# chaiyujin/sdfa-2019

Measured on AMD Instinct MI355X. Metric: animation frames/s/node (10 s@16 kHz clips); max|Δdgrad| vs CPU ref, higher is better.
Workload: dtype f32

## Files before the change

sdfa-2019_amd/csrc/api_core.cpp:

```cpp
#include "../../include/sdfa_stream.h"
#include "host.h"

#include <climits>
#include <cstdio>
#include <cstring>
#include <string>

static thread_local std::string g_err;

int sdfa_failv(int code, const char *fmt, va_list ap) {
    char buf[512];
    vsnprintf(buf, sizeof buf, fmt, ap);
    g_err = buf;
    return code;
}

int sdfa_fail(int code, const char *fmt, ...) {
    va_list ap;
    va_start(ap, fmt);
    sdfa_failv(code, fmt, ap);
    va_end(ap);
    return code;
}

thread_local int g_sdfa_mel_fft_radix4 = 0;
thread_local int g_sdfa_gather_plain_order = 0;
thread_local int g_sdfa_frontend_two_kernel = 0;
thread_local int g_sdfa_frontend_stream_block = 0;
thread_local int g_sdfa_frontend_stream_slots = 0;
thread_local int g_sdfa_frontend_stream_spin_max = 0;
thread_local int g_sdfa_frontend_stream_phases = 0;
thread_local int g_sdfa_frontend_t_major = 0;
extern thread_local int g_sdfa_gemm_variant;
thread_local int g_sdfa_freq_lstm_shape = 0;
thread_local int g_sdfa_pca_lds = 0;
thread_local int g_sdfa_pca_fp32 = 0;
thread_local int g_sdfa_conv_fp32 = 0;
thread_local int g_sdfa_time_lstm_split = 0;
thread_local int g_sdfa_time_lstm_handoff = 0;
thread_local int g_sdfa_time_lstm_timeout_us = 0;
thread_local int g_sdfa_share_gx0_off = 0;
thread_local int g_sdfa_encoder_dedup_off = 0;
thread_local int g_sdfa_attn_unfused = 0;

extern "C" {

int sdfa_abi_version(void) { return SDFA_ABI_VERSION; }
int sdfa_stream_abi_version(void) { return SDFA_STREAM_ABI_VERSION; }
const char *sdfa_last_error(void) { return g_err.c_str(); }

int sdfa_debug_set_option(const char *name, int value) {
    struct Option { const char *name; int *var; int lo = INT_MIN, hi = INT_MAX; const char *accepts = nullptr; };
    thread_local const Option options[] = {
        {"attn_unfused", &g_sdfa_attn_unfused},
        {"share_gx0_off", &g_sdfa_share_gx0_off},
        {"encoder_dedup_off", &g_sdfa_encoder_dedup_off},
        {"frontend_two_kernel", &g_sdfa_frontend_two_kernel},
        {"frontend_stream_phases", &g_sdfa_frontend_stream_phases},
        {"frontend_stream_spin_max", &g_sdfa_frontend_stream_spin_max, 0, INT_MAX, "0 (default) or a positive poll count"},
        {"frontend_stream_block", &g_sdfa_frontend_stream_block, 0, 256, "0 (default) or 1..256 frames"},
        {"frontend_stream_slots", &g_sdfa_frontend_stream_slots, 0, 256, "0 (default) or 1..256 workgroups per block"},
        {"gather_plain_order", &g_sdfa_gather_plain_order},
        {"mel_fft_radix4", &g_sdfa_mel_fft_radix4},
        {"frontend_t_major", &g_sdfa_frontend_t_major},
        {"time_lstm_timeout_us", &g_sdfa_time_lstm_timeout_us},
        {"time_lstm_handoff", &g_sdfa_time_lstm_handoff},
        {"time_lstm_split", &g_sdfa_time_lstm_split},
        {"gemm_variant", &g_sdfa_gemm_variant},
        {"freq_lstm_shape", &g_sdfa_freq_lstm_shape},
        {"pca_lds", &g_sdfa_pca_lds},
        {"conv_fp32", &g_sdfa_conv_fp32},
        {"pca_fp32", &g_sdfa_pca_fp32},
    };
    for (const Option &o : options)
        if (name && !strcmp(name, o.name)) {
            if (value < o.lo || value > o.hi) return sdfa_fail(SDFA_EINVAL, "%s: %s", o.name, o.accepts);
            *o.var = value;
            return SDFA_OK;
        }
    return sdfa_fail(SDFA_EINVAL, "unknown option '%s'", name ? name : "(null)");
}

}
```

sdfa-2019_amd/csrc/api_forward.cpp:

```cpp
#include "host.h"
#include "kernels.h"
#include "model.h"

#include <algorithm>

extern thread_local int g_sdfa_freq_lstm_shape, g_sdfa_pca_lds, g_sdfa_pca_fp32, g_sdfa_conv_fp32, g_sdfa_share_gx0_off, g_sdfa_attn_unfused, g_sdfa_encoder_dedup_off;

namespace {

constexpr int64_t CT_WORDS = 2048, CT_FLAGS = 16, ST_WORDS = SDFA_WS_STATUS_BYTES / 4;

struct Ws {
    int64_t P1, X3, HF, Z, GX, H0, H1, KP, QC, QP, ZK, SH, ZU, total;
    int64_t TRUNK, A0, A1, COEF;
    int64_t CT_FREQ, CT_PCA, CT_FLAG;
};

Ws layout(int64_t Nc, bool keep) {
    const int64_t Mc = 64 * Nc;
    Ws w{};
    int64_t o = 0;
    auto take = [&](int64_t n) { int64_t r = o; o += round_up(n, 64); return r; };
    take(ST_WORDS);
    if (keep) {
        w.P1 = take(2048 * Mc); w.X3 = take(2048 * Mc); w.HF = take((int64_t)HF_SLAB_ROWS * 4 * Mc); w.Z = take(256 * Mc);
        w.GX = take(2048 * Mc); w.H0 = take(512 * Mc); w.H1 = take(512 * Mc); w.KP = take(128 * Mc);
    } else {
        const int64_t A = take(2048 * Mc);
        const int64_t B = take(2048 * Mc);
        w.HF = take((int64_t)HF_SLAB_ROWS * 4 * Mc);
        w.P1 = A; w.GX = A;
        w.X3 = B; w.Z = B; w.H0 = B + 256 * Mc; w.H1 = B + 768 * Mc; w.KP = B + 1280 * Mc;
    }
    w.QC = take(512 * Nc); w.QP = take(128 * Nc); w.ZK = take(512 * Nc);
    const int64_t R = take(2560 * Nc);
    w.TRUNK = R; w.A0 = R + 512 * Nc; w.A1 = R + 1024 * Nc; w.COEF = R + 1280 * Nc;
    w.SH = take(sdfa_share_table_words(Nc) + 111);
    w.ZU = keep ? take(256 * Mc) : w.P1;
    const int64_t CT = take(CT_WORDS);
    w.CT_FREQ = CT; w.CT_PCA = CT + 1; w.CT_FLAG = CT + CT_FLAGS;
    w.total = o;
    return w;
}

int64_t capacity(int64_t bytes, bool keep) {
    const int64_t per128 = layout(128, keep).total * 4;
    int64_t nc = (bytes / per128 + 2) * 128;
    while (nc > 0 && layout(nc, keep).total * 4 > bytes) nc -= 128;
    return nc;
}

struct Prof {
    const sdfa_model *m;
    hipStream_t s;
    hipEvent_t pending = nullptr;
    void begin(const char *stage) {
        if (!m->profile) return;
        sdfa_model::Ev e; e.stage = stage;
        (void)hipEventCreate(&e.a); (void)hipEventCreate(&e.b);
        (void)hipEventRecord(e.a, s);
        pending = e.b;
        std::lock_guard<std::mutex> lk(m->ev_mu);
        m->events.push_back(e);
    }
    void end() {
        if (!m->profile || !pending) return;
        (void)hipEventRecord(pending, s);
        pending = nullptr;
    }
};

GemmArgs gemm_fc(const sdfa_model::Fc &fc, const float *Q, int64_t ldq, float *D, int64_t Nc, const int64_t *spk, int64_t nreal) {
    GemmArgs g = sdfa_gemm_k4(fc.w, fc.Ppad, Q, ldq, D, Nc, fc.K);
    g.bias = fc.b; g.cond_w = fc.cw; g.cond_idx = fc.cw ? spk : nullptr;
    g.Pstore = fc.Pstore; g.Qreal = nreal; g.act = fc.act;
    return g;
}

}

extern "C" {

int64_t sdfa_workspace_bytes(const sdfa_model *m, int64_t max_frames) {
    if (!m || max_frames <= 0) return sdfa_fail(SDFA_EINVAL, "workspace_bytes: bad argument");
    return layout(round_up(max_frames, 128), m->keep).total * 4;
}

int sdfa_debug_keep_intermediates(sdfa_model *m, int on) {
    if (!m) return sdfa_fail(SDFA_EINVAL, "null model");
    m->keep = on != 0;
    return SDFA_OK;
}

int sdfa_profile_enable(sdfa_model *m, int on) {
    if (!m) return sdfa_fail(SDFA_EINVAL, "null model");
    std::lock_guard<std::mutex> lk(m->ev_mu);
    m->profile = on != 0;
    for (auto &e : m->events) { (void)hipEventDestroy(e.a); (void)hipEventDestroy(e.b); }
    m->events.clear();
    return SDFA_OK;
}

float sdfa_profile_ms(const sdfa_model *m, const char *stage) {
    if (!m || !stage) return (float)sdfa_fail(SDFA_EINVAL, "profile_ms: bad argument");
    float total = 0.f;
    bool any = false;
    std::lock_guard<std::mutex> lk(m->ev_mu);
    for (auto &e : m->events)
        if (e.stage == stage) {
            float ms = 0.f;
            if (hipEventSynchronize(e.b) != hipSuccess || hipEventElapsedTime(&ms, e.a, e.b) != hipSuccess)
                return (float)sdfa_fail(SDFA_EHIP, "profile_ms: event query failed");
            total += ms; any = true;
        }
    return any ? total : (float)sdfa_fail(SDFA_EINVAL, "profile_ms: no such stage '%s'", stage);
}

int sdfa_profile_reset(sdfa_model *m) { return m ? sdfa_profile_enable(m, m->profile) : sdfa_fail(SDFA_EINVAL, "null model"); }

enum { STAGE_BODY = 0, STAGE_ATTENTION = 1, STAGE_REGRESSOR = 2 };
static int stage_terms(const sdfa_model *m, int stage) {
    switch (m->precision) {
    case SDFA_PREC_BF16_ATTENTION: return stage == STAGE_ATTENTION ? 1 : 0;
    case SDFA_PREC_BF16X3_ATTENTION: return stage == STAGE_ATTENTION ? 3 : 0;
    case SDFA_PREC_BF16X6: return 6;
    case SDFA_PREC_BF16X3: return 3;
    case SDFA_PREC_BF16: return 1;
    default: return 0;
    }
}

int sdfa_model_set_precision(sdfa_model *m, int mode) {
    if (!m) return sdfa_fail(SDFA_EINVAL, "null model");
    if (mode < SDFA_PREC_FP32 || mode > SDFA_PREC_BF16X6) return sdfa_fail(SDFA_EINVAL, "unknown precision mode %d", mode);
    m->precision = mode;
    return SDFA_OK;
}

int sdfa_model_precision(const sdfa_model *m) { return m ? m->precision : SDFA_EINVAL; }

int sdfa_model_set_reserved_cus(sdfa_model *m, int k) {
    if (!m) return sdfa_fail(SDFA_EINVAL, "null model");
    if (k < 0 || k > 128) return sdfa_fail(SDFA_EINVAL, "reserved_cus must be in [0, 128], got %d", k);
    m->reserved_cus.store(k);
    return SDFA_OK;
}

static int encoder_impl(const sdfa_model *m, const float *d_audio_feat, int64_t n_frames, const int32_t *d_frame_clip,
                        const int64_t *d_frame_start, int hop, float *d_z, float *d_align, void *d_workspace,
                        int64_t workspace_bytes, void *stream) {
    if (!m || !m->finalized) return sdfa_fail(SDFA_ESTATE, "encoder_forward: model not finalised");
    if (n_frames == 0) return SDFA_OK;
    if (!d_audio_feat || !d_z || !d_workspace || n_frames < 0) return sdfa_fail(SDFA_EINVAL, "encoder_forward: bad argument");
    if (((uintptr_t)d_workspace | (uintptr_t)d_audio_feat | (uintptr_t)d_z) & 15) return sdfa_fail(SDFA_EINVAL, "encoder_forward: pointers must be 16-byte aligned");
    if ((uintptr_t)d_align & 3) return sdfa_fail(SDFA_EINVAL, "encoder_forward: d_align must be 4-byte aligned");
    const int64_t cap = capacity(workspace_bytes, m->keep);
    if (cap < 128) return sdfa_fail(SDFA_ENOSPACE, "encoder_forward: workspace of %lld bytes holds no 128-frame chunk", (long long)workspace_bytes);
    hipStream_t s = (hipStream_t)stream;
    Prof pf{m, s};
    float *ws = (float *)d_workspace;
    for (int64_t f0 = 0; f0 < n_frames; f0 += cap) {
        const int64_t N = std::min(cap, n_frames - f0);
        const int64_t Nc = round_up(N, 128), Mc = 64 * Nc;
        const Ws w = layout(Nc, m->keep);
        ConvArgs ca{};
        ca.audio_feat = d_audio_feat + f0 * (64 * 128 * 3); ca.N = N; ca.Nc = Nc; ca.Mc = Mc;
        ca.w1 = m->w1; ca.b1 = m->b1; ca.s1 = m->s1; ca.t1 = m->t1; ca.P1 = ws + w.P1;
        ca.w2 = m->w2; ca.b2 = m->b2; ca.s2 = m->s2; ca.t2 = m->t2;
        ca.w3 = m->w3; ca.b3 = m->b3; ca.s3 = m->s3; ca.t3 = m->t3; ca.X3 = ws + w.X3;
        const bool table = d_frame_clip != nullptr;
        const bool share = table || (!m->keep && !g_sdfa_encoder_dedup_off);
        const int64_t *d_ulimit = nullptr;
        int32_t *col_to_u = nullptr;
        if (share) {
            ShareArgs sa{};
            sa.N = N; sa.Nc = Nc; sa.Mc = Mc;
            sdfa_share_carve(sa, reinterpret_cast<int32_t *>(ws + w.SH));
            pf.begin("share_map");
            if (table) {
                sa.frame_clip = d_frame_clip + f0; sa.frame_start = d_frame_start + f0; sa.hop = hop;
                sa.t_lo = 6; sa.t_hi = 58;
                HIP_TRY(sdfa_launch_share_map(sa, s));
            } else {
                sa.feat = ca.audio_feat;
                sa.hash = reinterpret_cast<uint64_t *>(ws + w.HF); sa.linked = sa.hash + Mc;
                HIP_TRY(sdfa_launch_share_map_content(sa, s));
            }
            pf.end();
            d_ulimit = sa.counts + 1; col_to_u = sa.col_to_u;
            ca.col_src = sa.col_src; ca.col_limit = d_ulimit;
        }
        const int conv_terms = g_sdfa_conv_fp32 ? 0 : stage_terms(m, STAGE_BODY);
        if (m->keep && conv_terms) {
            pf.begin("conv1"); HIP_TRY(sdfa_launch_conv1(ca, s)); pf.end();
            ca.wb = m->cv_wb; ca.terms = conv_terms;
            pf.begin("conv23"); HIP_TRY(sdfa_launch_conv123(ca, s)); pf.end();
        } else if (m->keep) {
            pf.begin("conv1"); HIP_TRY(sdfa_launch_conv1(ca, s)); pf.end();
            pf.begin("conv23"); HIP_TRY(sdfa_launch_conv23(ca, s)); pf.end();
        } else {
            ca.wb = m->cv_wb; ca.terms = conv_terms;
            pf.begin("conv23"); HIP_TRY(sdfa_launch_conv123(ca, s)); pf.end();
        }

        const int fl_terms = stage_terms(m, STAGE_BODY);
        FreqLstmArgs fa{ws + w.X3, m->fl_w, m->fl_b, ws + w.HF, Mc, d_ulimit, m->fl_wb, fl_terms, reinterpret_cast<int *>(ws + w.CT_FREQ),
                        g_sdfa_freq_lstm_shape ? g_sdfa_freq_lstm_shape : (fl_terms ? 0 : m->freq_shape.load()), m->reserved_cus.load()};
        pf.begin("freq_lstm"); HIP_TRY(sdfa_launch_freq_lstm(fa, s)); pf.end();

        GemmArgs g = sdfa_gemm_k4(m->fp_w, 256, ws + w.HF, Mc, ws + w.Z, Mc, 8192);
        g.bias = m->fp_b; g.q_tile_major = 1; g.q_slab_rows = HF_SLAB_ROWS;
        g.terms = stage_terms(m, STAGE_BODY);
        g.reserve_cus = m->reserved_cus.load();
        if (share) { g.D = ws + w.ZU; g.q_limit = d_ulimit; }
        pf.begin("freq_proj"); HIP_TRY(sdfa_launch_gemm(g, s)); pf.end();
        const bool share_gx0 = share && !m->keep && stage_terms(m, STAGE_BODY) == 0 && !g_sdfa_share_gx0_off;
        if (share && !share_gx0) {
            pf.begin("share_expand"); HIP_TRY(sdfa_launch_expand_cols(ws + w.ZU, col_to_u, ws + w.Z, 64, Mc, s)); pf.end();
        }

        const float *xin = share_gx0 ? ws + w.ZU : ws + w.Z;
        float *hout[2] = {ws + w.H0, ws + w.H1};
        const char *gxn[2] = {"gx0", "gx1"}, *lsn[2] = {"lstm0", "lstm1"};
        for (int l = 0; l < 2; ++l) {
            const bool mapped = share_gx0 && l == 0;
            float *gx = mapped ? ws + w.HF : ws + w.GX;
            GemmArgs gi = sdfa_gemm_k4(m->gx_w[l], 2048, xin, Mc, gx, Mc, l == 0 ? 256 : 512);
            gi.terms = stage_terms(m, STAGE_BODY);
            gi.reserve_cus = m->reserved_cus.load();
            if (mapped) gi.q_limit = d_ulimit;
            pf.begin(gxn[l]); HIP_TRY(sdfa_launch_gemm(gi, s)); pf.end();
            TimeLstmArgs ta{gx, m->tl_w[l], hout[l], Nc, Mc, m->tl_wb[l], stage_terms(m, STAGE_BODY),
                            reinterpret_cast<unsigned *>(ws + w.CT_FLAG), CT_WORDS - CT_FLAGS, m->tl_w16[l],
                            reinterpret_cast<unsigned *>(ws), m->reserved_cus.load(), mapped ? col_to_u : nullptr};
            pf.begin(lsn[l]); HIP_TRY(sdfa_launch_time_lstm(ta, s)); pf.end();
            xin = hout[l];
        }
        const int at_terms = stage_terms(m, STAGE_ATTENTION);
        const bool key_fused = g_sdfa_attn_unfused != 1;
        pf.begin("attn_proj");
        GemmArgs gk = sdfa_gemm_k4(m->kp_w, 128, ws + w.H1, Mc, ws + w.KP, Mc, 512);
        gk.terms = at_terms;
        if (!key_fused) HIP_TRY(sdfa_launch_gemm(gk, s));
        GemmArgs gc = sdfa_gemm_k4(m->qc_w, 512, ws + w.H1 + 31 * Nc * 4, Mc, ws + w.QC, Nc, 1536);
        gc.seg_k = 512; gc.seg_col = Nc; gc.terms = at_terms;
        HIP_TRY(sdfa_launch_gemm(gc, s));
        GemmArgs gq = sdfa_gemm_k4(m->qp_w, 128, ws + w.QC, Nc, ws + w.QP, Nc, 512);
        gq.terms = at_terms;
        HIP_TRY(sdfa_launch_gemm(gq, s));
        const bool tail_fused = key_fused && (at_terms == 0 || at_terms == 6) && g_sdfa_attn_unfused != 2 && sdfa_attn_fuses_tail(Nc, m->reserved_cus.load());
        if (key_fused) {
            AttnKeyArgs ak{};
            ak.Wk = m->kp_w; ak.H = ws + w.H1; ak.QP = ws + w.QP; ak.v = m->at_v; ak.b = m->at_b;
            ak.S = ws + w.KP;
            ak.Nc = Nc; ak.Mc = Mc; ak.terms = at_terms == 6 ? 0 : at_terms; ak.reserve_cus = m->reserved_cus.load();
            if (tail_fused) {
                ak.fuse_tail = 1; ak.Zk4 = ws + w.ZK; ak.z_out = d_z + f0 * 512; ak.align_out = d_align ? d_align + f0 * 64 : nullptr; ak.N = N;
            }
            HIP_TRY(sdfa_launch_attn_key_score(ak, s));
        }
        pf.end();

        AttnArgs aa{};
        aa.KP = ws + w.KP; aa.QP = ws + w.QP; aa.H = ws + w.H1; aa.v = m->at_v; aa.b = m->at_b;
        aa.Zk4 = ws + w.ZK; aa.z_out = d_z + f0 * 512; aa.align_out = d_align ? d_align + f0 * 64 : nullptr;
        aa.N = N; aa.Nc = Nc; aa.Mc = Mc;
        aa.S = key_fused ? ws + w.KP : nullptr;
        pf.begin("attn"); if (!tail_fused) HIP_TRY(sdfa_launch_attn(aa, s)); pf.end();
    }
    return SDFA_OK;
}

int sdfa_model_autotune(sdfa_model *m, int64_t n_frames, void *d_workspace, int64_t workspace_bytes, void *stream) {
    if (!m || !m->finalized) return sdfa_fail(SDFA_ESTATE, "autotune: model not finalised");
    if (!d_workspace || n_frames <= 0 || ((uintptr_t)d_workspace & 15)) return sdfa_fail(SDFA_EINVAL, "autotune: bad argument");
    const int64_t cap = capacity(workspace_bytes, m->keep);
    if (cap < 128) return sdfa_fail(SDFA_ENOSPACE, "autotune: workspace too small");
    const int64_t Nc = round_up(std::min(cap, n_frames), 128), Mc = 64 * Nc;
    const Ws w = layout(Nc, m->keep);
    float *ws = (float *)d_workspace;
    hipStream_t s = (hipStream_t)stream;
    HIP_TRY(hipMemsetAsync(ws + w.X3, 0, (size_t)2048 * Mc * sizeof(float), s));
    hipEvent_t e0, e1;
    HIP_TRY(hipEventCreate(&e0));
    HIP_TRY(hipEventCreate(&e1));
    static const int forms[] = {9, 8, 5, 3};
    float best_ms = 0.f;
    int best = m->freq_shape.load(), rc = SDFA_OK;
    for (int form : forms) {
        FreqLstmArgs fa{ws + w.X3, m->fl_w, m->fl_b, ws + w.HF, Mc, nullptr, m->fl_wb, 0, reinterpret_cast<int *>(ws + w.CT_FREQ), form, m->reserved_cus.load()};
        float ms = 0.f;
        for (int rep = 0; rep < 3 && rc == SDFA_OK; ++rep) {
            if (rep == 1 && hipEventRecord(e0, s) != hipSuccess) rc = SDFA_EHIP;
            if (sdfa_launch_freq_lstm(fa, s) != hipSuccess) rc = SDFA_EHIP;
        }
        if (rc == SDFA_OK && (hipEventRecord(e1, s) != hipSuccess || hipEventSynchronize(e1) != hipSuccess || hipEventElapsedTime(&ms, e0, e1) != hipSuccess)) rc = SDFA_EHIP;
        if (rc != SDFA_OK) break;
        if (best_ms == 0.f || ms < best_ms) { best_ms = ms; best = form; }
    }
    (void)hipEventDestroy(e0);
    (void)hipEventDestroy(e1);
    if (rc != SDFA_OK) return sdfa_fail(rc, "autotune: a HIP call failed: %s", hipGetErrorString(hipGetLastError()));
    m->freq_shape.store(best);
    return best;
}

int sdfa_encoder_forward(const sdfa_model *m, const float *d_audio_feat, int64_t n_frames, float *d_z, float *d_align,
                         void *d_workspace, int64_t workspace_bytes, void *stream) {
    return encoder_impl(m, d_audio_feat, n_frames, nullptr, nullptr, 0, d_z, d_align, d_workspace, workspace_bytes, stream);
}

int sdfa_encoder_forward_shared(const sdfa_model *m, const float *d_audio_feat, int64_t n_frames, const int32_t *d_frame_clip,
                                const int64_t *d_frame_start, int hop, float *d_z, float *d_align, void *d_workspace,
                                int64_t workspace_bytes, void *stream) {
    if (!d_frame_clip || !d_frame_start || hop <= 0) return sdfa_fail(SDFA_EINVAL, "encoder_forward_shared: frame table missing");
    return encoder_impl(m, d_audio_feat, n_frames, d_frame_clip, d_frame_start, hop, d_z, d_align, d_workspace, workspace_bytes, stream);
}

static hipError_t expand_rows(const sdfa_model *m, const float *coef, int64_t N, int64_t Nc, int64_t f0,
                              float *const *h_d_outs, int n_outs, int *queue, hipStream_t s) {
    float *d_out = h_d_outs[0];
    if (m->pca_n == 2) {
        PcaArgs pa{};
        pa.coef = coef; pa.basis_s = m->pca_q[0]; pa.basis_r = m->pca_q[1]; pa.mean_s = m->pca_bias[0]; pa.mean_r = m->pca_bias[1];
        pa.out = d_out + f0 * m->out_dim; pa.N = N; pa.Nc = Nc; pa.out_dim = m->out_dim;
        pa.n_extra = n_outs - 1;
        pa.reserve_cus = m->reserved_cus.load();
        pa.basis_b = m->pca_qb; pa.terms = (g_sdfa_pca_fp32 || m->precision != SDFA_PREC_BF16X3) ? 0 : 3;
        for (int x = 1; x < n_outs; ++x) pa.out_extra[x - 1] = h_d_outs[x] + f0 * m->out_dim;
        pa.ld_s = m->pca_ld[0]; pa.ld_r = m->pca_ld[1]; pa.cols_s = m->pca_cols[0]; pa.cols_r = m->pca_cols[1];
        if (g_sdfa_pca_lds != 4 && queue) return sdfa_launch_pca_dgrad_res(pa, queue, s);
        return sdfa_launch_pca_dgrad(pa, s);
    }
    for (int b = 0; b < m->pca_n; ++b) {
        GemmArgs g{};
        g.P = coef + (int64_t)m->pca_k0[b] * Nc; g.Q = m->pca_q[b]; g.D = d_out + f0 * m->out_dim;
        g.bias = m->pca_bias[b]; g.bias_on_q = 1;
        g.ldp = Nc; g.ldq = m->pca_ld[b]; g.ldd = m->out_dim; g.Ppad = Nc; g.Qpad = m->pca_ld[b]; g.Pstore = N;
        g.Qreal = m->pca_cols[b]; g.K = m->pca_K[b]; g.seg_k = g.K; g.act = ACT_NONE; g.out_mode = OUT_ROW;
        g.col_group = m->pca_group[b]; g.col_stride = 9; g.col_off = m->pca_off[b];
        g.n_extra = n_outs - 1;
        for (int x = 1; x < n_outs; ++x) g.D_extra[x - 1] = h_d_outs[x] + f0 * m->out_dim;
        g.terms = stage_terms(m, STAGE_REGRESSOR);
        hipError_t e = sdfa_launch_gemm(g, s);
        if (e != hipSuccess) return e;
    }
    return hipSuccess;
}

int sdfa_regress_forward(const sdfa_model *m, const float *d_z, const int64_t *d_speaker_id, int64_t n_frames,
                         float *d_coef, float *d_out, void *d_workspace, int64_t workspace_bytes, void *stream) {
    float *one[1] = {d_out};
    return sdfa_regress_forward_multi(m, d_z, d_speaker_id, n_frames, d_coef, one, d_out ? 1 : 0, d_workspace, workspace_bytes, stream);
}

int sdfa_regress_forward_multi(const sdfa_model *m, const float *d_z, const int64_t *d_speaker_id, int64_t n_frames,
                               float *d_coef, float *const *h_d_outs, int n_outs, void *d_workspace, int64_t workspace_bytes,
                               void *stream) {
    if (!m || !m->finalized) return sdfa_fail(SDFA_ESTATE, "regress_forward: model not finalised");
    if (n_outs < 0 || n_outs > SDFA_MAX_DESTS || (n_outs && !h_d_outs)) return sdfa_fail(SDFA_EINVAL, "regress_forward: 0..%d output destinations", SDFA_MAX_DESTS);
    for (int i = 0; i < n_outs; ++i) {
        if (!h_d_outs[i]) return sdfa_fail(SDFA_EINVAL, "regress_forward: output destination %d is null", i);
        if (m->head == SDFA_HEAD_DGRAD && ((uintptr_t)h_d_outs[i] & 15)) return sdfa_fail(SDFA_EINVAL, "regress_forward: d_out must be 16-byte aligned for the dgrad head");
        if ((uintptr_t)h_d_outs[i] & 3) return sdfa_fail(SDFA_EINVAL, "regress_forward: output pointers must be 4-byte aligned");
    }
    float *d_out = n_outs ? h_d_outs[0] : nullptr;
    if (n_frames == 0) return SDFA_OK;
    if (!d_z || !d_speaker_id || !d_workspace || n_frames < 0) return sdfa_fail(SDFA_EINVAL, "regress_forward: bad argument");
    if (((uintptr_t)d_workspace | (uintptr_t)d_z) & 15) return sdfa_fail(SDFA_EINVAL, "regress_forward: pointers must be 16-byte aligned");
    if (m->head == SDFA_HEAD_DGRAD && d_out && ((uintptr_t)d_out & 15)) return sdfa_fail(SDFA_EINVAL, "regress_forward: d_out must be 16-byte aligned for the dgrad head");
    if (((uintptr_t)d_out | (uintptr_t)d_coef) & 3) return sdfa_fail(SDFA_EINVAL, "regress_forward: output pointers must be 4-byte aligned");
    const int64_t cap = capacity(workspace_bytes, m->keep);
    if (cap < 128) return sdfa_fail(SDFA_ENOSPACE, "regress_forward: workspace too small");
    hipStream_t s = (hipStream_t)stream;
    Prof pf{m, s};
    float *ws = (float *)d_workspace;
    auto fcg = [m](const sdfa_model::Fc &fc, const float *Q, int64_t ldq, float *D, int64_t Nc, const int64_t *spk, int64_t nreal) {
        GemmArgs g = gemm_fc(fc, Q, ldq, D, Nc, spk, nreal);
        g.terms = stage_terms(m, STAGE_REGRESSOR);
        return g;
    };
    for (int64_t f0 = 0; f0 < n_frames; f0 += cap) {
        const int64_t N = std::min(cap, n_frames - f0);
        const int64_t Nc = round_up(N, 128);
        const Ws w = layout(Nc, m->keep);
        float *zk = ws + w.ZK, *trunk = ws + w.TRUNK, *a0 = ws + w.A0, *a1 = ws + w.A1, *coef = ws + w.COEF;
        const int64_t *spk = d_speaker_id + f0;
        pf.begin("mlp");
        HIP_TRY(sdfa_launch_rows_to_k4(d_z + f0 * 512, N, 512, zk, Nc, s));
        if (m->head == SDFA_HEAD_DGRAD) {
            HIP_TRY(sdfa_launch_gemm(fcg(m->trunk, zk, Nc, trunk, Nc, spk, N), s));
            for (int b = 0; b < 2; ++b) {
                HIP_TRY(sdfa_launch_gemm(fcg(m->br[b][0], trunk, Nc, a0, Nc, spk, N), s));
                HIP_TRY(sdfa_launch_gemm(fcg(m->br[b][1], a0, Nc, a1, Nc, spk, N), s));
                HIP_TRY(sdfa_launch_gemm(fcg(m->br[b][2], a1, Nc, coef + (b ? 96 * Nc : 0), Nc, spk, N), s));
            }
            if (d_coef) {
                HIP_TRY(sdfa_launch_k4_to_rows(coef, Nc, N, 288, 0, SDFA_COEF_SCALE, d_coef + f0 * m->coef_dim, m->coef_dim, s));
                HIP_TRY(sdfa_launch_k4_to_rows(coef, Nc, N, 288, 96, SDFA_COEF_ROTAT, d_coef + f0 * m->coef_dim + SDFA_COEF_SCALE, m->coef_dim, s));
            }
        } else {
            HIP_TRY(sdfa_launch_gemm(fcg(m->off[0], zk, Nc, a0, Nc, spk, N), s));
            HIP_TRY(sdfa_launch_gemm(fcg(m->off[1], a0, Nc, a1, Nc, spk, N), s));
            HIP_TRY(sdfa_launch_gemm(fcg(m->off[2], a1, Nc, coef, Nc, spk, N), s));
            if (d_coef) HIP_TRY(sdfa_launch_k4_to_rows(coef, Nc, N, 64, 0, SDFA_COEF_OFFSETS, d_coef + f0 * m->coef_dim, m->coef_dim, s));
        }
        pf.end();
        if (d_out) {
            pf.begin("pca");
            HIP_TRY(expand_rows(m, coef, N, Nc, f0, h_d_outs, n_outs, reinterpret_cast<int *>(ws + w.CT_PCA), s));
            pf.end();
        }
    }
    return SDFA_OK;
}

int sdfa_expand_coef(const sdfa_model *m, const float *d_coef, int64_t n_frames, float *d_out, void *d_workspace,
                     int64_t workspace_bytes, void *stream) {
    if (!m || !m->finalized) return sdfa_fail(SDFA_ESTATE, "expand_coef: model not finalised");
    if (n_frames == 0) return SDFA_OK;
    if (!d_coef || !d_out || !d_workspace || n_frames < 0) return sdfa_fail(SDFA_EINVAL, "expand_coef: bad argument");
    if ((uintptr_t)d_workspace & 15) return sdfa_fail(SDFA_EINVAL, "expand_coef: d_workspace must be 16-byte aligned");
    if (m->head == SDFA_HEAD_DGRAD && ((uintptr_t)d_out & 15)) return sdfa_fail(SDFA_EINVAL, "expand_coef: d_out must be 16-byte aligned for the dgrad head");
    if (((uintptr_t)d_out | (uintptr_t)d_coef) & 3) return sdfa_fail(SDFA_EINVAL, "expand_coef: pointers must be 4-byte aligned");
    const int64_t cap = capacity(workspace_bytes, m->keep);
    if (cap < 128) return sdfa_fail(SDFA_ENOSPACE, "expand_coef: workspace too small");
    hipStream_t s = (hipStream_t)stream;
    Prof pf{m, s};
    float *ws = (float *)d_workspace;
    for (int64_t f0 = 0; f0 < n_frames; f0 += cap) {
        const int64_t N = std::min(cap, n_frames - f0);
        const int64_t Nc = round_up(N, 128);
        const Ws w = layout(Nc, m->keep);
        float *coef = ws + w.COEF;
        const float *src = d_coef + f0 * m->coef_dim;
        pf.begin("pca");
        if (m->head == SDFA_HEAD_DGRAD) {
            HIP_TRY(sdfa_launch_rows_seg_to_k4(src, m->coef_dim, N, 0, SDFA_COEF_SCALE, coef, Nc, 0, 96, s));
            HIP_TRY(sdfa_launch_rows_seg_to_k4(src, m->coef_dim, N, SDFA_COEF_SCALE, SDFA_COEF_ROTAT, coef, Nc, 96, 192, s));
        } else {
            HIP_TRY(sdfa_launch_rows_seg_to_k4(src, m->coef_dim, N, 0, SDFA_COEF_OFFSETS, coef, Nc, 0, 64, s));
        }
        float *outs[1] = {d_out};
        HIP_TRY(expand_rows(m, coef, N, Nc, f0, outs, 1, reinterpret_cast<int *>(ws + w.CT_PCA), s));
        pf.end();
    }
    return SDFA_OK;
}

int64_t sdfa_debug_distinct_columns(const sdfa_model *m, int64_t n_frames, const void *d_workspace, void *stream) {
    if (!m || n_frames <= 0 || !d_workspace) return sdfa_fail(SDFA_EINVAL, "debug_distinct_columns: bad argument");
    const Ws w = layout(round_up(n_frames, 128), m->keep);
    int64_t counts[2] = {0, 0};
    HIP_TRY(hipMemcpyAsync(counts, (const float *)d_workspace + w.SH, sizeof counts, hipMemcpyDeviceToHost, (hipStream_t)stream));
    HIP_TRY(hipStreamSynchronize((hipStream_t)stream));
    return counts[0];
}

int sdfa_workspace_init(void *d_workspace, int64_t workspace_bytes, void *stream) {
    if (!d_workspace || workspace_bytes < SDFA_WS_STATUS_BYTES || ((uintptr_t)d_workspace & 15)) return sdfa_fail(SDFA_EINVAL, "workspace_init: bad argument");
    HIP_TRY(hipMemsetAsync(d_workspace, 0, SDFA_WS_STATUS_BYTES, (hipStream_t)stream));
    return SDFA_OK;
}

int sdfa_workspace_status_async(const void *d_workspace, uint32_t *h_status, void *stream) {
    if (!d_workspace || !h_status) return sdfa_fail(SDFA_EINVAL, "workspace_status_async: bad argument");
    HIP_TRY(hipMemcpyAsync(h_status, d_workspace, SDFA_WS_STATUS_WORDS * sizeof(uint32_t), hipMemcpyDeviceToHost, (hipStream_t)stream));
    return SDFA_OK;
}

int64_t sdfa_workspace_status(const void *d_workspace, int word, void *stream) {
    if (!d_workspace || word < 0 || word >= SDFA_WS_STATUS_WORDS) return sdfa_fail(SDFA_EINVAL, "workspace_status: bad argument");
    uint32_t v = 0;
    HIP_TRY(hipMemcpyAsync(&v, reinterpret_cast<const uint32_t *>(d_workspace) + word, sizeof v, hipMemcpyDeviceToHost, (hipStream_t)stream));
    HIP_TRY(hipStreamSynchronize((hipStream_t)stream));
    return (int64_t)v;
}

int sdfa_debug_tap(const sdfa_model *m, int what, int64_t n_frames, float *d_dst, const void *d_workspace, void *stream) {
    if (!m || !m->keep) return sdfa_fail(SDFA_ESTATE, "debug_tap needs sdfa_debug_keep_intermediates(model, 1) before the forward");
    if (what < 0 || what > 3 || n_frames <= 0 || !d_dst || !d_workspace) return sdfa_fail(SDFA_EINVAL, "debug_tap: bad argument");
    const int64_t Nc = round_up(n_frames, 128);
    const Ws w = layout(Nc, true);
    const float *ws = (const float *)d_workspace;
    const float *src = what == 0 ? ws + w.P1 : what == 1 ? ws + w.X3 : what == 2 ? ws + w.Z : ws + w.H1;
    HIP_TRY(sdfa_launch_tap(src, what, n_frames, Nc, d_dst, (hipStream_t)stream));
    return SDFA_OK;
}

}
```

sdfa-2019_amd/csrc/kernels.h:

```cpp
#pragma once
#include <hip/hip_runtime.h>
#include <stdint.h>

enum { ACT_NONE = 0, ACT_LRELU = 1, ACT_TANH = 2 };

constexpr int HF_SLAB_ROWS = 2048;
enum { OUT_K4 = 0, OUT_ROW = 1 };
constexpr int SDFA_MAX_DESTS = 8;

struct GemmArgs {
    const float *P;
    const float *Q;
    float *D;
    const float *bias;
    const float *cond_w;
    const int64_t *cond_idx;
    int64_t ldp, ldq, ldd;
    int64_t Ppad, Qpad;
    int64_t Pstore;
    int64_t Qreal;
    int K;
    int seg_k;
    int64_t seg_col;
    int act, out_mode, bias_on_q;
    int terms;
    int q_tile_major;
    int q_slab_rows;
    const int64_t *q_limit;
    int col_group, col_stride, col_off;
    float *D_extra[SDFA_MAX_DESTS - 1];
    int n_extra;
    int reserve_cus;
};
hipError_t sdfa_launch_gemm(const GemmArgs &a, hipStream_t s);
inline GemmArgs sdfa_gemm_k4(const float *P, int64_t rows, const float *Q, int64_t ldq, float *D, int64_t cols, int K) {
    GemmArgs g{};
    g.P = P; g.Q = Q; g.D = D;
    g.ldp = rows; g.Ppad = rows; g.Pstore = rows;
    g.ldq = ldq; g.ldd = cols; g.Qpad = cols; g.Qreal = cols;
    g.K = K; g.seg_k = K; g.act = ACT_NONE; g.out_mode = OUT_K4;
    return g;
}

struct PcaArgs {
    const float *coef;
    const float *basis_s, *basis_r;
    const float *mean_s, *mean_r;
    float *out;
    int64_t N, Nc, out_dim, ld_s, ld_r, cols_s, cols_r;
    float *out_extra[SDFA_MAX_DESTS - 1];
    int n_extra;
    int reserve_cus;
    const void *basis_b;
    int terms;
};
hipError_t sdfa_launch_pca_dgrad(const PcaArgs &a, hipStream_t s);
hipError_t sdfa_launch_pca_dgrad_res(const PcaArgs &a, int *queue, hipStream_t s);

struct FrontendConsts {
    const float *hamm;
    const float2 *twiddle;
    const int *mel_bin0;
    const float *mel_w8;
    int win, hop, sliding, nbins_used, nnz;
};
hipError_t sdfa_launch_frontend(const FrontendConsts &c, const float *pcm, const int64_t *clip_off,
                                const int64_t *clip_len, const int32_t *frame_clip, const int64_t *frame_start,
                                int64_t n_frames, float *audio_feat, hipStream_t s);
hipError_t sdfa_launch_mel_columns(const FrontendConsts &c, const float *pcm, const int64_t *clip_off, const int64_t *clip_len,
                                   const int32_t *frame_clip, const int64_t *frame_start, const int32_t *col_src,
                                   const int64_t *n_distinct, float *mel_table, hipStream_t s);
hipError_t sdfa_launch_mel_stream(const FrontendConsts &c, const float *pcm, const int64_t *clip_off, const int64_t *clip_len,
                                  const int32_t *frame_clip, const int64_t *frame_start, const int32_t *prev, const int32_t *shift,
                                  int64_t n_frames, int block, int slots, int producer_consumer, int spin_max, int *status, float *audio_feat, hipStream_t s);
hipError_t sdfa_launch_mel_ring(const FrontendConsts &c, const float *rings, int r, int n_rings, const int64_t *view_ring, const int64_t *view_hi,
                                const int32_t *frame_view, const int64_t *frame_start, const int32_t *prev, const int32_t *shift, int64_t n_frames,
                                int block, int slots, int producer_consumer, int spin_max, int *status, float *audio_feat, hipStream_t s);
hipError_t sdfa_launch_ring_append(float *rings, int r, int n_rings, const int64_t *seg, int n_seg, const float *src, int64_t n_src, hipStream_t s);
hipError_t sdfa_launch_gather_features(const float *mel_table, const int32_t *col_to_u, int64_t n_frames, int64_t Nc, int frame_major,
                                       float *audio_feat, hipStream_t s);

struct ConvArgs {
    const float *audio_feat;
    int64_t N, Nc, Mc;
    const float *w1, *b1, *s1, *t1;
    float *P1;
    const float *w2, *b2, *s2, *t2;
    const float *w3, *b3, *s3, *t3;
    float *X3;
    const int32_t *col_src;
    const int64_t *col_limit;
    const void *wb;
    int terms;
};
hipError_t sdfa_launch_conv1(const ConvArgs &a, hipStream_t s);
hipError_t sdfa_launch_conv23(const ConvArgs &a, hipStream_t s);
hipError_t sdfa_launch_conv123(const ConvArgs &a, hipStream_t s);

struct FreqLstmArgs {
    const float *X3;
    const float *W;
    const float *bias;
    float *HF;
    int64_t Mc;
    const int64_t *col_limit;
    const void *Wb;
    int terms;
    int *tile_counter;
    int shape;
    int reserve_cus;
};
hipError_t sdfa_launch_freq_lstm(const FreqLstmArgs &a, hipStream_t s);

struct TimeLstmArgs {
    const float *GX;
    const float *W;
    float *H;
    int64_t Nc, Mc;
    const void *Wb;
    int terms;
    unsigned *flags;
    int64_t flag_words;
    const float *W16;
    unsigned *status;
    int reserve_cus;
    const int32_t *col_map;
};
hipError_t sdfa_launch_time_lstm(const TimeLstmArgs &a, hipStream_t s);

struct AttnArgs {
    const float *KP;
    const float *QP;
    const float *H;
    const float *v;
    const float *b;
    float *Zk4;
    float *z_out;
    float *align_out;
    int64_t N, Nc, Mc;
    const float *S;
};
hipError_t sdfa_launch_attn(const AttnArgs &a, hipStream_t s);

struct AttnKeyArgs {
    const float *Wk;
    const float *H;
    const float *QP;
    const float *v, *b;
    float *S;
    int64_t Nc, Mc;
    int terms;
    int reserve_cus;
    int ts_shift;
    int fuse_tail;
    float *Zk4, *z_out, *align_out;
    int64_t N;
};
bool sdfa_attn_fuses_tail(int64_t Nc, int reserve_cus);
hipError_t sdfa_launch_attn_key_score(const AttnKeyArgs &a, hipStream_t s);

hipError_t sdfa_launch_rows_to_k4(const float *src, int64_t N, int F, float *dst, int64_t ld, hipStream_t s);
hipError_t sdfa_launch_rows_seg_to_k4(const float *src, int64_t src_ld, int64_t N, int c0, int nf, float *dst, int64_t ld,
                                      int f0, int nf_pad, hipStream_t s);
hipError_t sdfa_launch_k4_to_rows(const float *src, int64_t ld, int64_t N, int F, int f0, int nf, float *dst,
                                  int64_t dst_ld, hipStream_t s);
hipError_t sdfa_launch_tap(const float *src, int what, int64_t N, int64_t Nc, float *dst, hipStream_t s);

struct ShareArgs {
    const int32_t *frame_clip;
    const int64_t *frame_start;
    int hop;
    int t_lo, t_hi;
    int frame_major;
    int64_t N, Nc, Mc;
    int32_t *prev, *shift;
    int32_t *owner, *flag, *uid;
    int32_t *tile_sum;
    int32_t *col_src;
    int32_t *col_to_u;
    int64_t *counts;
    const float *feat;
    uint64_t *hash;
    uint64_t *linked;
};
inline int64_t sdfa_share_table_words(int64_t Nc) { return 16 + 2 * Nc + 5 * (64 * Nc) + (64 * Nc) / 1024 + 1; }
inline void sdfa_share_carve(ShareArgs &a, int32_t *base) {
    a.counts = reinterpret_cast<int64_t *>(base);
    a.prev = base + 16; a.shift = a.prev + a.Nc;
    a.owner = a.shift + a.Nc; a.flag = a.owner + a.Mc; a.uid = a.flag + a.Mc;
    a.col_src = a.uid + a.Mc; a.col_to_u = a.col_src + a.Mc; a.tile_sum = a.col_to_u + a.Mc;
}
hipError_t sdfa_launch_share_map(const ShareArgs &a, hipStream_t s);
hipError_t sdfa_launch_share_map_content(const ShareArgs &a, hipStream_t s);
hipError_t sdfa_launch_share_prev(const ShareArgs &a, hipStream_t s);
hipError_t sdfa_launch_expand_cols(const float *Zu, const int32_t *col_to_u, float *Z, int nquads, int64_t Mc, hipStream_t s);

struct MeshArgs {
    const float *dgrad;
    int64_t n_frames;
    int n_tris, n_verts, n_free, free_pad;
    int n_src_tris;
    const int64_t *seek_src;
    const float *seek_w;
    const float *reg_xt;
    const int *inc_ptr;
    const int *inc_tri;
    const float *inc_coef;
    const int *vert_col;
    const float *tmpl;
    float *rhs;
    const float *sol;
    float *verts;
    int64_t ld;
};
hipError_t sdfa_launch_mesh_rhs(const MeshArgs &a, hipStream_t s);
hipError_t sdfa_launch_mesh_scatter(const MeshArgs &a, hipStream_t s);
hipError_t sdfa_launch_seek_plan(const int32_t *tslist, const int64_t *frame_off, const int64_t *query_off, int n_clips, double fps,
                                 int64_t n_queries, int64_t *src, float *w, hipStream_t s);
hipError_t sdfa_launch_seek_rows(const float *rows, int64_t width, const int64_t *src, const float *w, int64_t nq, float *out, hipStream_t s);
struct DgradArgs {
    const float *src;
    const float *target;
    const uint32_t *faces;
    const uint8_t *mask;
    int64_t n_frames;
    int n_tris, n_verts, target_is_offsets;
    double eps;
    float *out32;
    double *out64;
};
hipError_t sdfa_launch_deform_grad(const DgradArgs &a, hipStream_t s);
hipError_t sdfa_launch_ensemble_mean(const float *a, const float *b, int64_t n, float *out, hipStream_t s);

struct ResampleArgs {
    const float *x;
    int64_t n_in;
    float *y;
    int64_t n_res, n_out;
    const double *win, *delta;
    const double *treg;
    int64_t nwin, step;
    double scale;
    int num_table;
};
hipError_t sdfa_launch_resample(const ResampleArgs &a, hipStream_t s);
```

sdfa-2019_amd/csrc/share.hip:

```cpp
#include "common.h"
#include "kernels.h"

namespace {


__global__ void share_prev_kernel(ShareArgs a) {
    const int64_t n = (int64_t)blockIdx.x * blockDim.x + threadIdx.x;
    if (n >= a.Nc) return;
    int prev = -1, shift = 0;
    if (n < a.N) {
        const int clip = a.frame_clip[n];
        const int64_t s = a.frame_start[n];
        for (int back = 1; back <= 64 && n - back >= 0; ++back) {
            const int64_t q = n - back;
            if (a.frame_clip[q] != clip) break;
            const int64_t diff = s - a.frame_start[q];
            if (diff <= 0) break;
            if (diff > (int64_t)(a.t_hi - a.t_lo) * a.hop) break;
            if (diff % a.hop == 0) { prev = (int)q; shift = (int)(diff / a.hop); break; }
        }
    }
    a.prev[n] = prev;
    a.shift[n] = shift;
}

__device__ __forceinline__ int64_t col_index(const ShareArgs &a, int64_t n, int t) { return a.frame_major ? n * 64 + t : (int64_t)t * a.Nc + n; }
__device__ __forceinline__ void col_of(const ShareArgs &a, int64_t i, int64_t &n, int &t) {
    if (a.frame_major) { n = i >> 6; t = (int)(i & 63); } else { n = i % a.Nc; t = (int)(i / a.Nc); }
}

__global__ void share_owner_kernel(ShareArgs a) {
    const int64_t i = (int64_t)blockIdx.x * blockDim.x + threadIdx.x;
    if (i >= a.Mc) return;
    int64_t n;
    int t;
    col_of(a, i, n, t);
    if (n >= a.N) { a.owner[i] = -1; a.flag[i] = 0; return; }
    while (t >= a.t_lo && t <= a.t_hi) {
        const int p = a.prev[n];
        if (p < 0) break;
        const int tt = t + a.shift[n];
        if (tt > a.t_hi) break;
        n = p; t = tt;
    }
    const int64_t o = col_index(a, n, t);
    a.owner[i] = (int)o;
    a.flag[i] = o == i ? 1 : 0;
}

constexpr int COL_QUADS = 96;

__device__ __forceinline__ uint64_t mix64(uint64_t x) {
    x ^= x >> 32; x *= 0xd6e8feb86659fd93ull;
    x ^= x >> 32; x *= 0xd6e8feb86659fd93ull;
    return x ^ (x >> 32);
}

__global__ __launch_bounds__(256) void share_hash_kernel(ShareArgs a) {
    const int l = threadIdx.x & 31;
    const int64_t col = ((int64_t)blockIdx.x * 256 + threadIdx.x) >> 5, M = a.N * 64;
    uint64_t h = 0;
    if (col < M) {
        const uint4 *row = reinterpret_cast<const uint4 *>(a.feat) + col * COL_QUADS;
#pragma unroll
        for (int j = 0; j < 3; ++j) {
            const int q = l + 32 * j;
            const uint4 v = row[q];
            const uint64_t lo = (uint64_t)v.x | (uint64_t)v.y << 32, hi = (uint64_t)v.z | (uint64_t)v.w << 32;
            h += mix64(lo + 0x9e3779b97f4a7c15ull * (uint64_t)(2 * q + 1)) + mix64(hi + 0x9e3779b97f4a7c15ull * (uint64_t)(2 * q + 2));
        }
    }
    for (int off = 16; off; off >>= 1) h += __shfl_xor(h, off);
    if (col < M && l == 0) a.hash[col] = mix64(h) | 1;
}

constexpr int MATCH_SLOTS = 128;
__global__ __launch_bounds__(256) void share_match_kernel(ShareArgs a) {
    __shared__ unsigned long long hn[4][64], tab[4][MATCH_SLOTS];
    const int w = threadIdx.x >> 6, lane = threadIdx.x & 63;
    const int64_t n = (int64_t)blockIdx.x * 4 + w;
    const bool real = n < a.N && n > 0;
    const unsigned long long mine = real ? a.hash[n * 64 + lane] : 1;
    hn[w][lane] = mine;
    tab[w][lane] = 0; tab[w][lane + 64] = 0;
    __syncthreads();
    for (int slot = (int)(mine >> 8) & (MATCH_SLOTS - 1), k = 0; k < MATCH_SLOTS; ++k, slot = (slot + 1) & (MATCH_SLOTS - 1)) {
        const unsigned long long old = atomicCAS(&tab[w][slot], 0ull, mine);
        if (old == 0 || old == mine) break;
    }
    __syncthreads();
    if (n >= a.Nc) return;
    int best = 0, bp = -1, bd = 0;
    if (real) {
        const int64_t lo = n > 64 ? n - 64 : 0;
        unsigned long long hp = a.hash[(n - 1) * 64 + lane];
        for (int64_t p = n - 1; p >= lo && best < 63; --p) {
            const unsigned long long hq = p > lo ? a.hash[(p - 1) * 64 + lane] : 0;
            bool member = false;
            for (int slot = (int)(hp >> 8) & (MATCH_SLOTS - 1), k = 0; k < MATCH_SLOTS; ++k, slot = (slot + 1) & (MATCH_SLOTS - 1)) {
                const unsigned long long v = tab[w][slot];
                if (v == hp) member = true;
                if (v == hp || v == 0) break;
            }
            if (__ballot(member)) {
                for (int d0 = 1; d0 < 64 - best; d0 += 4) {
                    int c[4];
#pragma unroll
                    for (int k = 0; k < 4; ++k) {
                        const int d = d0 + k;
                        const bool eq = lane >= d && hn[w][lane >= d ? lane - d : 0] == hp;
                        c[k] = __popcll(__ballot(eq));
                    }
#pragma unroll
                    for (int k = 0; k < 4; ++k)
                        if (c[k] > best) { best = c[k]; bp = (int)p; bd = d0 + k; }
                }
            }
            hp = hq;
        }
    }
    if (lane == 0) { a.prev[n] = bp; a.shift[n] = bd; }
}

__global__ __launch_bounds__(256) void share_verify_kernel(ShareArgs a) {
    const int64_t n = blockIdx.x;
    const int w = threadIdx.x >> 6, lane = threadIdx.x & 63, half = lane >> 5, l = lane & 31;
    const int p = a.prev[n], d = a.shift[n];
    unsigned bits = 0;
    if (p >= 0) {
        const uint64_t *hn = a.hash + n * 64, *hp = a.hash + (int64_t)p * 64;
        const uint4 *fn = reinterpret_cast<const uint4 *>(a.feat) + n * 64 * COL_QUADS;
        const uint4 *fp = reinterpret_cast<const uint4 *>(a.feat) + (int64_t)p * 64 * COL_QUADS;
        for (int j = 0; j < 8; ++j) {
            const int t = 16 * w + 2 * j + half, tt = t + d;
            const bool cand = tt < 64 && hn[t] == hp[tt];
            bool differ = false;
            if (cand) {
#pragma unroll
                for (int k = 0; k < 3; ++k) {
                    const uint4 x = fn[t * COL_QUADS + l + 32 * k], y = fp[tt * COL_QUADS + l + 32 * k];
                    differ |= ((x.x ^ y.x) | (x.y ^ y.y) | (x.z ^ y.z) | (x.w ^ y.w)) != 0;
                }
            }
            const uint64_t c = __ballot(cand), bad = __ballot(differ);
            if ((c & 1) && !(bad & 0xffffffffull)) bits |= 1u << (2 * j);
            if ((c >> 32 & 1) && !(bad >> 32)) bits |= 1u << (2 * j + 1);
        }
    }
    if (lane == 0) reinterpret_cast<uint16_t *>(a.linked)[n * 4 + w] = (uint16_t)bits;
}

__global__ void share_owner_content_kernel(ShareArgs a) {
    const int64_t i = (int64_t)blockIdx.x * blockDim.x + threadIdx.x;
    if (i >= a.Mc) return;
    int64_t n;
    int t;
    col_of(a, i, n, t);
    if (n >= a.N) { a.owner[i] = -1; a.flag[i] = 0; return; }
    while (t < 63 && (a.linked[n] >> t & 1)) {
        t += a.shift[n];
        n = a.prev[n];
    }
    const int64_t o = col_index(a, n, t);
    a.owner[i] = (int)o;
    a.flag[i] = o == i ? 1 : 0;
}

__device__ __forceinline__ int block_inclusive_scan_1024(int v, int *part) {
    const int tid = threadIdx.x;
    part[tid] = v;
    __syncthreads();
    for (int off = 1; off < 1024; off <<= 1) {
        const int x = tid >= off ? part[tid - off] : 0;
        __syncthreads();
        part[tid] += x;
        __syncthreads();
    }
    return part[tid];
}

__global__ __launch_bounds__(1024) void share_scan_tiles_kernel(ShareArgs a) {
    __shared__ int part[1024];
    const int64_t i = (int64_t)blockIdx.x * 1024 + threadIdx.x;
    const int f = i < a.Mc ? a.flag[i] : 0;
    const int inc = block_inclusive_scan_1024(f, part);
    if (i < a.Mc) a.uid[i] = inc - f;
    if (threadIdx.x == 1023) a.tile_sum[blockIdx.x] = inc;
}

__global__ __launch_bounds__(1024) void share_scan_sums_kernel(ShareArgs a, int ntiles) {
    __shared__ int part[1024];
    int carry = 0;
    for (int base = 0; base < ntiles; base += 1024) {
        const int t = base + threadIdx.x;
        const int v = t < ntiles ? a.tile_sum[t] : 0;
        const int inc = block_inclusive_scan_1024(v, part);
        if (t < ntiles) a.tile_sum[t] = carry + inc - v;
        carry += part[1023];
        __syncthreads();
    }
    if (threadIdx.x == 0) {
        const int64_t mu = carry, pad = (mu + 255) / 256 * 256;
        a.counts[0] = mu;
        a.counts[1] = pad;
    }
}

__global__ __launch_bounds__(1024) void share_scan_fix_kernel(ShareArgs a) {
    const int64_t i = (int64_t)blockIdx.x * 1024 + threadIdx.x;
    const int64_t mu = a.counts[0], pad = a.counts[1];
    if (i < a.Mc) {
        const int u = a.uid[i] + a.tile_sum[blockIdx.x];
        a.uid[i] = u;
        int64_t n;
        int t;
        col_of(a, i, n, t);
        if (a.flag[i]) a.col_src[u] = (int)(n * 64 + t);
    }
    if (i >= mu && i < pad) a.col_src[i] = -1;
}

__global__ void share_assign_kernel(ShareArgs a) {
    const int64_t m = (int64_t)blockIdx.x * blockDim.x + threadIdx.x;
    if (m >= a.Mc) return;
    const int o = a.owner[m];
    a.col_to_u[m] = o >= 0 ? a.uid[o] : 0;
}

__global__ void expand_cols_kernel(const float4 *__restrict__ Zu, const int32_t *__restrict__ col_to_u, float4 *__restrict__ Z,
                                   int nquads, int64_t Mc) {
    const int64_t m = (int64_t)blockIdx.x * blockDim.x + threadIdx.x;
    if (m >= Mc) return;
    const int64_t u = col_to_u[m];
    for (int q = 0; q < nquads; ++q) Z[(int64_t)q * Mc + m] = Zu[(int64_t)q * Mc + u];
}

}

static void launch_share_numbering(const ShareArgs &a, hipStream_t s) {
    const int ntiles = (int)((a.Mc + 1023) / 1024);
    hipLaunchKernelGGL(share_scan_tiles_kernel, dim3(ntiles), dim3(1024), 0, s, a);
    hipLaunchKernelGGL(share_scan_sums_kernel, dim3(1), dim3(1024), 0, s, a, ntiles);
    hipLaunchKernelGGL(share_scan_fix_kernel, dim3(ntiles), dim3(1024), 0, s, a);
    hipLaunchKernelGGL(share_assign_kernel, dim3((unsigned)((a.Mc + 255) / 256)), dim3(256), 0, s, a);
}

hipError_t sdfa_launch_share_map_content(const ShareArgs &a, hipStream_t s) {
    hipLaunchKernelGGL(share_hash_kernel, dim3((unsigned)(a.N * 8)), dim3(256), 0, s, a);
    hipLaunchKernelGGL(share_match_kernel, dim3((unsigned)(a.Nc / 4)), dim3(256), 0, s, a);
    hipLaunchKernelGGL(share_verify_kernel, dim3((unsigned)a.N), dim3(256), 0, s, a);
    hipLaunchKernelGGL(share_owner_content_kernel, dim3((unsigned)((a.Mc + 255) / 256)), dim3(256), 0, s, a);
    launch_share_numbering(a, s);
    return hipGetLastError();
}

hipError_t sdfa_launch_share_map(const ShareArgs &a, hipStream_t s) {
    hipLaunchKernelGGL(share_prev_kernel, dim3((unsigned)((a.Nc + 255) / 256)), dim3(256), 0, s, a);
    hipLaunchKernelGGL(share_owner_kernel, dim3((unsigned)((a.Mc + 255) / 256)), dim3(256), 0, s, a);
    launch_share_numbering(a, s);
    return hipGetLastError();
}

hipError_t sdfa_launch_share_prev(const ShareArgs &a, hipStream_t s) {
    hipLaunchKernelGGL(share_prev_kernel, dim3((unsigned)((a.Nc + 255) / 256)), dim3(256), 0, s, a);
    return hipGetLastError();
}

hipError_t sdfa_launch_expand_cols(const float *Zu, const int32_t *col_to_u, float *Z, int nquads, int64_t Mc, hipStream_t s) {
    hipLaunchKernelGGL(expand_cols_kernel, dim3((unsigned)((Mc + 255) / 256)), dim3(256), 0, s,
                       reinterpret_cast<const float4 *>(Zu), col_to_u, reinterpret_cast<float4 *>(Z), nquads, Mc);
    return hipGetLastError();
}
```

Baseline: 141,500.

## Split freq_proj GEMM tail wave into a finer-grained tail kernel

The share scan now also computes a q_full boundary that rounds the unique-column count down to a whole number of persistent-grid waves when the leftover partial wave is small. The main freq_proj GEMM stops at q_full, and a new 64x64-tile MFMA tail kernel covers the remaining columns up to the padded limit. The goal is to avoid the load imbalance of a mostly-empty last wave of 256-wide tiles. In exchange it adds one extra kernel launch, and the tail kernel's grid is sized by the host upper bound, so surplus workgroups start and then exit early.

```diff
diff --git a/sdfa-2019_amd/csrc/api_core.cpp b/sdfa-2019_amd/csrc/api_core.cpp
--- a/sdfa-2019_amd/csrc/api_core.cpp
+++ b/sdfa-2019_amd/csrc/api_core.cpp
@@ -41,6 +41,7 @@
 thread_local int g_sdfa_time_lstm_timeout_us = 0;
 thread_local int g_sdfa_share_gx0_off = 0;
 thread_local int g_sdfa_encoder_dedup_off = 0;
+thread_local int g_sdfa_freq_proj_tail = 0;
 thread_local int g_sdfa_attn_unfused = 0;
 
 extern "C" {
@@ -55,6 +56,7 @@
         {"attn_unfused", &g_sdfa_attn_unfused},
         {"share_gx0_off", &g_sdfa_share_gx0_off},
         {"encoder_dedup_off", &g_sdfa_encoder_dedup_off},
+        {"freq_proj_tail", &g_sdfa_freq_proj_tail, 0, 2, "0 (rule), 1 (never) or 2 (always)"},
         {"frontend_two_kernel", &g_sdfa_frontend_two_kernel},
         {"frontend_stream_phases", &g_sdfa_frontend_stream_phases},
         {"frontend_stream_spin_max", &g_sdfa_frontend_stream_spin_max, 0, INT_MAX, "0 (default) or a positive poll count"},
diff --git a/sdfa-2019_amd/csrc/api_forward.cpp b/sdfa-2019_amd/csrc/api_forward.cpp
--- a/sdfa-2019_amd/csrc/api_forward.cpp
+++ b/sdfa-2019_amd/csrc/api_forward.cpp
@@ -1,10 +1,12 @@
+#include "common.h"
 #include "host.h"
 #include "kernels.h"
 #include "model.h"
 
 #include <algorithm>
 
-extern thread_local int g_sdfa_freq_lstm_shape, g_sdfa_pca_lds, g_sdfa_pca_fp32, g_sdfa_conv_fp32, g_sdfa_share_gx0_off, g_sdfa_attn_unfused, g_sdfa_encoder_dedup_off;
+extern thread_local int g_sdfa_gemm_variant, g_sdfa_freq_lstm_shape, g_sdfa_pca_lds, g_sdfa_pca_fp32, g_sdfa_conv_fp32, g_sdfa_share_gx0_off, g_sdfa_attn_unfused, g_sdfa_encoder_dedup_off,
+    g_sdfa_freq_proj_tail;
 
 namespace {
 
@@ -172,10 +174,18 @@
         const bool share = table || (!m->keep && !g_sdfa_encoder_dedup_off);
         const int64_t *d_ulimit = nullptr;
         int32_t *col_to_u = nullptr;
+        bool split_tail = false;
+        int64_t fat_grid = 0;
+        const int64_t *d_qfull = nullptr;
         if (share) {
             ShareArgs sa{};
             sa.N = N; sa.Nc = Nc; sa.Mc = Mc;
             sdfa_share_carve(sa, reinterpret_cast<int32_t *>(ws + w.SH));
+            split_tail = !m->keep && stage_terms(m, STAGE_BODY) == 0 && g_sdfa_gemm_variant == 0 && Mc / 256 >= 512 && g_sdfa_freq_proj_tail != 1;
+            if (split_tail) {
+                fat_grid = sdfa_fat_grid(256, Mc, sdfa_cu_count(), m->reserved_cus.load());
+                sa.fat_grid = (int)fat_grid; sa.tail_mode = g_sdfa_freq_proj_tail;
+            }
             pf.begin("share_map");
             if (table) {
                 sa.frame_clip = d_frame_clip + f0; sa.frame_start = d_frame_start + f0; sa.hop = hop;
@@ -187,7 +197,7 @@
                 HIP_TRY(sdfa_launch_share_map_content(sa, s));
             }
             pf.end();
-            d_ulimit = sa.counts + 1; col_to_u = sa.col_to_u;
+            d_ulimit = sa.counts + 1; d_qfull = sa.counts + 2; col_to_u = sa.col_to_u;
             ca.col_src = sa.col_src; ca.col_limit = d_ulimit;
         }
         const int conv_terms = g_sdfa_conv_fp32 ? 0 : stage_terms(m, STAGE_BODY);
@@ -212,8 +222,14 @@
         g.bias = m->fp_b; g.q_tile_major = 1; g.q_slab_rows = HF_SLAB_ROWS;
         g.terms = stage_terms(m, STAGE_BODY);
         g.reserve_cus = m->reserved_cus.load();
-        if (share) { g.D = ws + w.ZU; g.q_limit = d_ulimit; }
-        pf.begin("freq_proj"); HIP_TRY(sdfa_launch_gemm(g, s)); pf.end();
+        if (share) { g.D = ws + w.ZU; g.q_limit = split_tail ? d_qfull : d_ulimit; }
+        pf.begin("freq_proj");
+        HIP_TRY(sdfa_launch_gemm(g, s));
+        if (split_tail) {
+            GemmTailArgs gt{m->fp_w, ws + w.HF, m->fp_b, ws + w.ZU, Mc, HF_SLAB_ROWS, d_qfull, d_ulimit, (int)fat_grid - 1};
+            HIP_TRY(sdfa_launch_gemm_tail(gt, s));
+        }
+        pf.end();
         const bool share_gx0 = share && !m->keep && stage_terms(m, STAGE_BODY) == 0 && !g_sdfa_share_gx0_off;
         if (share && !share_gx0) {
             pf.begin("share_expand"); HIP_TRY(sdfa_launch_expand_cols(ws + w.ZU, col_to_u, ws + w.Z, 64, Mc, s)); pf.end();
diff --git a/sdfa-2019_amd/csrc/gemm_tail.hip b/sdfa-2019_amd/csrc/gemm_tail.hip
--- /dev/null
+++ b/sdfa-2019_amd/csrc/gemm_tail.hip
@@ -0,0 +1,69 @@
+#include "common.h"
+#include "kernels.h"
+
+namespace {
+
+constexpr int TAIL_K = 8192, TAIL_ROWS = 256, KQ = 8, TB = 64;
+
+__global__ __launch_bounds__(256, 4) void gemm_tail_kernel(GemmTailArgs a) {
+    __shared__ float4 sP[2][KQ][TB], sQ[2][KQ][TB];
+    const int tid = threadIdx.x, lane = tid & 63, wave = tid >> 6;
+    const int wp = wave >> 1, wq = wave & 1, l31 = lane & 31, h = lane >> 5;
+    const int64_t q_lo = *a.q_lo, q_hi = std::min<int64_t>(*a.q_hi, a.ldd);
+    const int64_t q0 = q_lo + (int64_t)(blockIdx.x >> 2) * TB;
+    const int p0 = (blockIdx.x & 3) * TB;
+    if (q_lo < 0 || q0 >= q_hi) return;
+
+    const float4 *__restrict__ P = reinterpret_cast<const float4 *>(a.P) + p0;
+    const float4 *__restrict__ Q = reinterpret_cast<const float4 *>(a.Q) + (q0 >> 7) * (int64_t)a.q_slab_rows * 128 + (q0 & 127);
+    const int r = tid >> 6, c = tid & 63;
+    constexpr int nstage = TAIL_K / 32;
+
+    f32x16 acc;
+#pragma unroll
+    for (int i = 0; i < 16; ++i) acc[i] = 0.f;
+
+    float4 rp0, rp1, rq0, rq1;
+#define TAIL_GLOAD(st)                                                                      \
+    {                                                                                       \
+        rp0 = P[((st) * KQ + r) * TAIL_ROWS + c]; rp1 = P[((st) * KQ + r + 4) * TAIL_ROWS + c]; \
+        rq0 = Q[((st) * KQ + r) * 128 + c];       rq1 = Q[((st) * KQ + r + 4) * 128 + c];   \
+    }
+#define TAIL_LSTORE(buf) { sP[buf][r][c] = rp0; sP[buf][r + 4][c] = rp1; sQ[buf][r][c] = rq0; sQ[buf][r + 4][c] = rq1; }
+    TAIL_GLOAD(0)
+    TAIL_LSTORE(0)
+    __syncthreads();
+    for (int st = 0; st < nstage; ++st) {
+        const int buf = st & 1;
+        const bool more = st + 1 < nstage;
+        if (more) TAIL_GLOAD(st + 1)
+#pragma unroll
+        for (int kb = 0; kb < KQ / 2; ++kb) {
+            const float4 fa = sP[buf][2 * kb + h][wp * 32 + l31], fb = sQ[buf][2 * kb + h][wq * 32 + l31];
+            mfma4(acc, fa, fb);
+        }
+        if (more) TAIL_LSTORE(buf ^ 1)
+        __syncthreads();
+    }
+#undef TAIL_GLOAD
+#undef TAIL_LSTORE
+
+    const int64_t q = q0 + wq * 32 + l31;
+#pragma unroll
+    for (int g = 0; g < 4; ++g) {
+        const int p = p0 + wp * 32 + 8 * g + 4 * h;
+        float v[4] = {acc[4 * g + 0], acc[4 * g + 1], acc[4 * g + 2], acc[4 * g + 3]};
+        const float4 b = ld4(a.bias + p);
+        v[0] += b.x; v[1] += b.y; v[2] += b.z; v[3] += b.w;
+        st4(a.D + ((p / 4) * a.ldd + q) * 4, make_float4(v[0], v[1], v[2], v[3]));
+    }
+}
+
+}
+
+hipError_t sdfa_launch_gemm_tail(const GemmTailArgs &a, hipStream_t s) {
+    if (!a.P || !a.Q || !a.D || !a.bias || !a.q_lo || !a.q_hi || a.q_slab_rows < TAIL_K / 4 || a.ldd % 256) return hipErrorInvalidValue;
+    if (a.max_tiles <= 0) return hipSuccess;
+    hipLaunchKernelGGL(gemm_tail_kernel, dim3((unsigned)a.max_tiles * 16), dim3(256), 0, s, a);
+    return hipGetLastError();
+}
diff --git a/sdfa-2019_amd/csrc/kernels.h b/sdfa-2019_amd/csrc/kernels.h
--- a/sdfa-2019_amd/csrc/kernels.h
+++ b/sdfa-2019_amd/csrc/kernels.h
@@ -182,6 +182,8 @@
     const float *feat;
     uint64_t *hash;
     uint64_t *linked;
+    int fat_grid;
+    int tail_mode;
 };
 inline int64_t sdfa_share_table_words(int64_t Nc) { return 16 + 2 * Nc + 5 * (64 * Nc) + (64 * Nc) / 1024 + 1; }
 inline void sdfa_share_carve(ShareArgs &a, int32_t *base) {
@@ -194,6 +196,20 @@
 hipError_t sdfa_launch_share_map_content(const ShareArgs &a, hipStream_t s);
 hipError_t sdfa_launch_share_prev(const ShareArgs &a, hipStream_t s);
 hipError_t sdfa_launch_expand_cols(const float *Zu, const int32_t *col_to_u, float *Z, int nquads, int64_t Mc, hipStream_t s);
+
+struct GemmTailArgs {
+    const float *P, *Q, *bias;
+    float *D;
+    int64_t ldd;
+    int q_slab_rows;
+    const int64_t *q_lo, *q_hi;
+    int max_tiles;
+};
+hipError_t sdfa_launch_gemm_tail(const GemmTailArgs &a, hipStream_t s);
+inline int64_t sdfa_fat_grid(int64_t rows, int64_t cols, int cus, int reserve_cus) {
+    const int64_t ntiles = (rows / 256) * (cols / 256), wgs = cus - reserve_cus > 1 ? cus - reserve_cus : 1;
+    return ntiles < wgs ? ntiles : wgs;
+}
 
 struct MeshArgs {
     const float *dgrad;
diff --git a/sdfa-2019_amd/csrc/share.hip b/sdfa-2019_amd/csrc/share.hip
--- a/sdfa-2019_amd/csrc/share.hip
+++ b/sdfa-2019_amd/csrc/share.hip
@@ -188,6 +188,7 @@
     if (threadIdx.x == 1023) a.tile_sum[blockIdx.x] = inc;
 }
 
+constexpr int TAIL_NUM = 3, TAIL_DEN = 4;
 __global__ __launch_bounds__(1024) void share_scan_sums_kernel(ShareArgs a, int ntiles) {
     __shared__ int part[1024];
     int carry = 0;
@@ -203,6 +204,12 @@
         const int64_t mu = carry, pad = (mu + 255) / 256 * 256;
         a.counts[0] = mu;
         a.counts[1] = pad;
+        int64_t q_full = pad;
+        if (a.fat_grid > 0 && a.tail_mode != 1) {
+            const int64_t T = pad / 256, G = a.fat_grid, r = T % G;
+            if (a.tail_mode == 2 || r * TAIL_DEN <= G * TAIL_NUM) q_full = (T - r) * 256;
+        }
+        a.counts[2] = q_full;
     }
 }
 
```

Result: faster. 144,600, median of 6 (+2.2%).
